# rsasaki0109/lidarslam_ros2

Hardware: AMD Instinct MI355X
Metric: scan registrations/sec (30k-pt scan vs 10-frame submap) (higher is better)
Workload: dtype f32; 1 GPU; cfg2: single NDT align(), 30000-pt VLP-32 scan (vg 0.2) vs 10-frame submap (vg 0.1), ndt_resolution 5.0, DIRECT7, max_iterations 30, transformation_epsilon 0; 1018 different scans (stream of 64); target_points=661519, voxels_valid=643, derivative_passes_last_scan=242, parallelism=1 registration stream per GPU x1, collective=none (one rank)

## Files before the change

### lidarslam_ros2_amd/csrc/ndt.hip

```cpp
#include "ndt.hpp"

#include <cmath>
#include <cstdlib>
#include <type_traits>

#include "grid_device.hpp"
#include "ndt_canon.hpp"
#include "ndt_point.hpp"
#include "sort.hpp"
#include "voxel_device.hpp"

namespace lsr {

namespace {

__host__ __device__ inline void angle_tables(const double* p, bool with_hessian, int d1_sign, float* jang, float* hang) {
  double cx, cy, cz, sx, sy, sz;
  if (fabs(p[3]) < 10e-5) { cx = 1.0; sx = 0.0; } else { cx = cos(p[3]); sx = sin(p[3]); }
  if (fabs(p[4]) < 10e-5) { cy = 1.0; sy = 0.0; } else { cy = cos(p[4]); sy = sin(p[4]); }
  if (fabs(p[5]) < 10e-5) { cz = 1.0; sz = 0.0; } else { cz = cos(p[5]); sz = sin(p[5]); }
  jang[0] = (float)(-sx * sz + cx * sy * cz); jang[1] = (float)(-sx * cz - cx * sy * sz); jang[2] = (float)(-cx * cy);
  jang[3] = (float)(cx * sz + sx * sy * cz);  jang[4] = (float)(cx * cz - sx * sy * sz);  jang[5] = (float)(-sx * cy);
  jang[6] = (float)(-sy * cz);                jang[7] = (float)(sy * sz);                 jang[8] = (float)(cy);
  jang[9] = (float)(sx * cy * cz);            jang[10] = (float)(-sx * cy * sz);          jang[11] = (float)(sx * sy);
// ... 598 lines not shown
    const long long _t3 = (long long)wall_clock64(), _c3 = (long long)clock64();         \
    unsigned long long* _r = (unsigned long long*)&g_lsr_timing[(810 + ((hess) ? 1 : 0)) * 32]; \
    atomicAdd(&_r[0], 1ull); atomicAdd(&_r[1], (unsigned long long)(_p_t1 - _p_t0)); atomicAdd(&_r[2], (unsigned long long)(_p_t2 - _p_t7)); \
    atomicAdd(&_r[3], (unsigned long long)(_t3 - _p_t2)); atomicAdd(&_r[4], (unsigned long long)(_c3 - _p_c0)); atomicAdd(&_r[5], (unsigned long long)(_t3 - _p_t0)); \
  }
#else
#define LSR_STAMP(k)
#define LSR_STAMP_T(k, t)
#define LSR_SPAN_BEGIN(seq)
#define LSR_SPAN_END(seq)
#define LSR_CTL_BEGIN(L)
#define LSR_CTL_END(col)
#define LSR_PASS_BEGIN()
#define LSR_PASS_MARK(var)
#define LSR_PASS_END(hess)
#endif

__device__ __forceinline__ int uniform_i(int v) { return __builtin_amdgcn_readfirstlane(v); }
__device__ __forceinline__ float uniform_f(float v) { return __int_as_float(__builtin_amdgcn_readfirstlane(__float_as_int(v))); }
__device__ __forceinline__ double uniform_d(double v) {
  const int lo = __builtin_amdgcn_readfirstlane(__double2loint(v)), hi = __builtin_amdgcn_readfirstlane(__double2hiint(v));
  return __hiloint2double(hi, lo);
}




__device__ __forceinline__ float dpp_quad_sum(float v) {
  v += __int_as_float(__builtin_amdgcn_update_dpp(0, __float_as_int(v), 0xB1, 0xF, 0xF, true));
  v += __int_as_float(__builtin_amdgcn_update_dpp(0, __float_as_int(v), 0x4E, 0xF, 0xF, true));
  return v;
}

template <int NOFF, int TAB, int PTS, bool KD = false>
__global__ __launch_bounds__(4 * PTS) void ndt_eval_quad_kernel(const NdtProblem P, const int seq) {
  constexpr int THREADS = 4 * PTS;
  constexpr int PITCH_PT = PTS + 8, PITCH_O = PTS + 4;
  constexpr int NT = (NOFF + 3) / 4;
  static_assert(PTS % 64 == 0, "a workgroup batch is a whole number of canonical chunks");
  if ((int)blockIdx.x >= P.nblocks) return;
  const int tid = threadIdx.x, ql = tid & 3, pq = tid >> 2;
  LSR_STAMP(0)
  LSR_STAMP_T(9, THREADS - 64)
  LSR_PASS_BEGIN()
  LSR_SPAN_BEGIN(seq)

  __shared__ float s_pt[14][PITCH_PT];
  __shared__ __attribute__((aligned(16))) float s_o[29][PITCH_O];
  __shared__ double s_bin[NDT_NBINS][32];
  __shared__ unsigned long long s_ibin[NDT_NBINS * 32];
  __shared__ double s_sum[NDT_NRED];
  __shared__ double s_lu[8][2];
  constexpr int STATE_Q = (int)(sizeof(NdtState) / 16);
  __shared__ uint4 s_state_q[STATE_Q];
  unsigned int* s_state = reinterpret_cast<unsigned int*>(s_state_q);
  extern __shared__ uint4 s_table[];

  const NdtState* __restrict__ Sin = P.st + (seq & 1);
  NdtState* __restrict__ Sout = P.st + ((seq + 1) & 1);

  const int stride = P.nblocks * PTS;
  int i = blockIdx.x * PTS + pq;
  float x = 0.f, y = 0.f, z = 0.f;
  unsigned int ang_entry = 0u, ang_entry_b = 0u;
  {
    const uint4* gq = reinterpret_cast<const uint4*>(Sin);
    const uint4 stq = (tid < STATE_Q) ? gq[tid] : make_uint4(0u, 0u, 0u, 0u);
    long long msum = 0;
    if (seq > 0 && tid < NDT_NBINS * 32) {
      const long long* b = P.bins + (size_t)((seq + 2) % NDT_NBANKS) * NDT_BANK_WORDS + tid;
      long long m[NDT_NSHARDS];
#pragma unroll
      for (int sh = 0; sh < NDT_NSHARDS; sh++) m[sh] = b[sh * (NDT_NBINS * 32)];
      msum = ((m[0] + m[1]) + (m[2] + m[3])) + ((m[4] + m[5]) + (m[6] + m[7]));
    }
    if (tid < NDT_NBINS * 32) {
      const int k = tid >> 5;
      s_bin[k][tid & 31] = canon::bin_value(msum, k);
      s_ibin[tid] = 0ull;
    }
    if (tid < STATE_Q) s_state_q[tid] = stq;
    if (i < P.n) { x = P.sx[i]; y = P.sy[i]; z = P.sz[i]; }
    if (tid < 64) ang_entry = k_angle_entries[tid];
    if (tid < 8) ang_entry_b = k_angle_entries[64 + tid];
  }
  LSR_STAMP_T(8, 0)
  LSR_STAMP_T(10, THREADS - 64)
  barrier_lds_only();
  LdsState* L = (LdsState*)s_state;
  LSR_STAMP(1)
  LSR_PASS_MARK(_p_t1)
  if (P.mailbox != nullptr && blockIdx.x == 0 && tid == 0)
    __hip_atomic_store(&P.mailbox->progress, ((unsigned long long)(unsigned int)L->token << 32) | (unsigned int)seq,
                       __ATOMIC_RELAXED, __HIP_MEMORY_SCOPE_SYSTEM);
  if (uniform_i(L->done)) {
    if (blockIdx.x == 0 && seq > 0) {
      uint4* gq = reinterpret_cast<uint4*>(Sout);
      if (tid < STATE_Q) gq[tid] = s_state_q[tid];
    }
    return;
  }
  if (TAB == NDT_TAB_LDS) {
    const int nchunks = P.lds_bytes >> 10;
    const unsigned char* img = reinterpret_cast<const unsigned char*>(P.lds_image) + (size_t)(tid & 63) * 16;
    unsigned char* dst = reinterpret_cast<unsigned char*>(s_table);
    if (tid >= 64)
      for (int c = (tid >> 6) - 1; c < nchunks; c += THREADS / 64 - 1)
        __builtin_amdgcn_global_load_lds((const __attribute__((address_space(1))) void*)(img + (size_t)c * 1024),
                                         (__attribute__((address_space(3))) void*)(dst + (size_t)c * 1024), 16, 0, 0);
  }
  if (tid < 64) {
    if (seq > 0) {
      if (tid < NDT_NRED) {
        const double b4 = s_bin[4][tid], b3 = s_bin[3][tid], b2 = s_bin[2][tid], b1 = s_bin[1][tid], b0 = s_bin[0][tid];
        double t = canon::fold(b0, b1, b2, b3, b4);
        if (s_bin[0][31] != 0.0 || s_bin[1][31] != 0.0) t = canon::poisoned();
        s_sum[tid] = t;
      }
      wave_lds_fence();
      LSR_STAMP(6)
      LSR_CTL_BEGIN(L)
      ndt_controller_wave0(L, (const LdsDouble*)s_sum);
      wave_lds_fence();
      LSR_CTL_END(0)
      LSR_STAMP(5)
      build_request_wave0(reinterpret_cast<NdtState*>(s_state), &s_lu[0][0], reinterpret_cast<float*>(&s_lu[4][0]), ang_entry, ang_entry_b);
      LSR_CTL_END(2)
      LSR_STAMP(4)
    }
    if (blockIdx.x == 0) {
      uint4* gq = reinterpret_cast<uint4*>(Sout);
      gq[tid] = s_state_q[tid];
      if (tid + 64 < STATE_Q) gq[tid + 64] = s_state_q[tid + 64];
    }
  }
  __syncthreads();
  if (uniform_i(L->done)) {
    if (P.mailbox != nullptr && blockIdx.x == 0 && tid == 0) {
      NdtMailbox* mb = P.mailbox;
#pragma unroll
      for (int k = 0; k < 16; k++) mb->final_T[k] = L->final_T[k];
      mb->converged = L->converged;
      mb->nr_iterations = L->nr_iterations;
      mb->n_evals = L->n_evals;
      mb->n_passes = L->n_passes;
      mb->trans_probability = L->trans_probability;
      mb->last_pairs = L->last_pairs;
      __threadfence_system();
      __hip_atomic_store(&mb->done, (unsigned int)L->token, __ATOMIC_RELEASE, __HIP_MEMORY_SCOPE_SYSTEM);
    }
    return;
  }
  if (blockIdx.x == 0) {
    uint4* zb = reinterpret_cast<uint4*>(P.bins + (size_t)((seq + 1) % NDT_NBANKS) * NDT_BANK_WORDS);
    for (int k = tid; k < NDT_BANK_WORDS / 2; k += THREADS) zb[k] = make_uint4(0u, 0u, 0u, 0u);
  }
  LSR_STAMP(7)
  LSR_PASS_MARK(_p_t7)

  const int form = uniform_i(L->want_hessian);
  const bool hess = form != NDT_PASS_GRAD;
  const bool fused = form == NDT_PASS_FUSED;
  const double d1d = uniform_d(L->d1);
  const float d2 = uniform_f((float)L->d2);
  float T[12];
#pragma unroll
  for (int k = 0; k < 12; k++) T[k] = uniform_f(L->T[k]);
  const float leaf = P.leaf;
  LSR_STAMP(11)

  const unsigned short* s_map = reinterpret_cast<const unsigned short*>(s_table);
  const float4* s_rec = reinterpret_cast<const float4*>(reinterpret_cast<const unsigned char*>(s_table) + P.lds_map_bytes);

  long long* const bank = P.bins + (size_t)(seq % NDT_NBANKS) * NDT_BANK_WORDS + (size_t)(blockIdx.x & (NDT_NSHARDS - 1)) * (NDT_NBINS * 32);
  const bool one_batch = (long long)blockIdx.x * PTS + stride >= (long long)P.n;
  for (int base = blockIdx.x * PTS; base < P.n; base += stride) {
    {
      const float tx = xform_ref(T[0], T[1], T[2], T[3], x, y, z);
      const float ty = xform_ref(T[4], T[5], T[6], T[7], x, y, z);
      const float tz = xform_ref(T[8], T[9], T[10], T[11], x, y, z);
      const float fx = floorf(tx / leaf), fy = floorf(ty / leaf), fz = floorf(tz / leaf);
      const bool finite_ok = (i < P.n) && (fabsf(fx) < 1.0e9f) && (fabsf(fy) < 1.0e9f) && (fabsf(fz) < 1.0e9f);
      const int ci = finite_ok ? (int)fx : INT_MIN / 2, cj = finite_ok ? (int)fy : INT_MIN / 2, ck = finite_ok ? (int)fz : INT_MIN / 2;

      bool valid[NT], score_only[NT];
      int cellv[NT];
#pragma unroll
      for (int t = 0; t < NT; t++) {
        score_only[t] = false;
        const int o = ql + 4 * t;
        int dx, dy, dz;
        Offsets<NOFF>::get(o, dx, dy, dz);
        const int a = ci + dx, b = cj + dy, c = ck + dz;
        const bool in = (o < NOFF) & (a >= P.min_b[0]) & (a <= P.max_b[0]) & (b >= P.min_b[1]) & (b <= P.max_b[1]) &
                        (c >= P.min_b[2]) & (c <= P.max_b[2]);
        valid[t] = in;
        cellv[t] = in ? ((a - P.min_b[0]) + (b - P.min_b[1]) * P.mul1 + (c - P.min_b[2]) * P.mul2) : 0;
      }
      if (KD) {
#pragma unroll
        for (int t = 0; t < NT; t++) {
          const int code = valid[t] ? P.cell_slot[cellv[t]] : -1, sl = kd_slot(code);
          const float4 cen = P.centroid[sl >= 0 ? sl : 0];
          valid[t] = (sl >= 0) & centroid_in_radius(tx, ty, tz, cen.x, cen.y, cen.z, P.radius2);
          score_only[t] = valid[t] & (code < -1);
        }
      }
      float4 r0[NT], r1[NT], r2[NT];
      if (TAB == NDT_TAB_LDS) {
        int slot[NT];
#pragma unroll
        for (int t = 0; t < NT; t++) {
          const int sl = (int)s_map[cellv[t]];
          valid[t] = valid[t] & (sl != 0xFFFF);
          slot[t] = valid[t] ? sl : 0;
        }
#pragma unroll
        for (int t = 0; t < NT; t++) {
          r0[t] = s_rec[slot[t] * 3 + 0];
          r1[t] = s_rec[slot[t] * 3 + 1];
          r2[t] = s_rec[slot[t] * 3 + 2];
        }
      } else {
        size_t ridx[NT];
#pragma unroll
        for (int t = 0; t < NT; t++) {
// ... 6 lines not shown
          }
        }
#pragma unroll
        for (int t = 0; t < NT; t++) {
          r0[t] = P.rec[ridx[t] * 4 + 0];
          r1[t] = P.rec[ridx[t] * 4 + 1];
          r2[t] = P.rec[ridx[t] * 4 + 2];
        }
      }

      if (KD) {
#pragma unroll
        for (int t = 0; t < NT; t++) {
          if (score_only[t]) {
            valid[t] = true;
            r0[t] = r1[t] = r2[t] = make_float4(0.f, 0.f, 0.f, 0.f);
          }
        }
      }
      float score = 0.f, npairs = 0.f;
      float A0 = 0.f, A1 = 0.f, A2 = 0.f;
      float E00 = 0.f, E01 = 0.f, E02 = 0.f, E11 = 0.f, E12 = 0.f, E22 = 0.f;
#pragma unroll
      for (int t = 0; t < NT; t++)
        pair_terms(valid[t], hess, tx, ty, tz, r0[t], r1[t], r2[t], d2, d1d, score, npairs, A0, A1, A2, E00, E01, E02, E11, E12, E22);
      score = dpp_quad_sum(score); npairs = dpp_quad_sum(npairs);
      A0 = dpp_quad_sum(A0); A1 = dpp_quad_sum(A1); A2 = dpp_quad_sum(A2);
      if (hess) {
        E00 = dpp_quad_sum(E00); E01 = dpp_quad_sum(E01); E02 = dpp_quad_sum(E02);
        E11 = dpp_quad_sum(E11); E12 = dpp_quad_sum(E12); E22 = dpp_quad_sum(E22);
        const float row0 = (ql == 0) ? score : (ql == 1) ? npairs : (ql == 2) ? A0 : A1;
        const float row1 = (ql == 0) ? A2 : (ql == 1) ? E00 : (ql == 2) ? E01 : E02;
        const float row2 = (ql == 0) ? E11 : (ql == 1) ? E12 : (ql == 2) ? E22 : x;
        s_pt[ql][pq] = row0;
        s_pt[4 + ql][pq] = row1;
        s_pt[8 + ql][pq] = row2;
        if (ql < 2) s_pt[12 + ql][pq] = (ql == 0) ? y : z;
      } else {
        float o[29];
        if (npairs != 0.f) {
          point_terms(false, x, y, z, score, npairs, A0, A1, A2, 0.f, 0.f, 0.f, 0.f, 0.f, 0.f, L->jang, L->hang, o);
        } else {
#pragma unroll
          for (int k = 0; k < NDT_NRED_GRAD; k++) o[k] = 0.f;
        }
        s_o[ql][pq] = (ql == 0) ? o[0] : (ql == 1) ? o[1] : (ql == 2) ? o[2] : o[3];
        s_o[4 + ql][pq] = (ql == 0) ? o[4] : (ql == 1) ? o[5] : (ql == 2) ? o[6] : o[7];
      }
      i += stride;
      x = 0.f; y = 0.f; z = 0.f;
      if (i < P.n) { x = P.sx[i]; y = P.sy[i]; z = P.sz[i]; }
    }
    LSR_STAMP(12)
    barrier_lds_only();
    if (hess) {
      if (tid < PTS) {
        const float npairs = s_pt[1][tid];
        float o[29];
        if (npairs != 0.f) {
          point_terms(true, s_pt[11][tid], s_pt[12][tid], s_pt[13][tid], s_pt[0][tid], npairs, s_pt[2][tid], s_pt[3][tid], s_pt[4][tid],
                      s_pt[5][tid], s_pt[6][tid], s_pt[7][tid], s_pt[8][tid], s_pt[9][tid], s_pt[10][tid], L->jang, L->hang, o);
        } else {
#pragma unroll
          for (int k = 0; k < 29; k++) o[k] = 0.f;
        }
#pragma unroll
        for (int k = 0; k < 29; k++) s_o[k][tid] = o[k];
      }
      LSR_STAMP(13)
      barrier_lds_only();
    }
    LSR_STAMP(14)
    if (!hess || fused) {
      constexpr int RUNS = PTS / 8;
      if (tid < NDT_NRED_GRAD * RUNS) {
        const int v = tid / RUNS, k = tid & 7;
        const double t = canon::reduce_grad(&s_o[v][8 * (tid % RUNS)]);
        bool poison;
        long long m = canon::piece(t, k < NDT_NBINS ? k : 0, &poison);
        int pz = poison ? 1 : 0;
        if (PTS == 128) { m += (long long)__shfl_xor((int)m, 8, 64); pz |= __shfl_xor(pz, 8, 64); }
        if ((tid & (RUNS - 1)) < NDT_NBINS) {
          unsigned long long* dst = one_batch ? reinterpret_cast<unsigned long long*>(bank) : s_ibin;
          if (m != 0) atomicAdd(dst + k * 32 + v, (unsigned long long)m);
          if (pz && k == 0) atomicAdd(dst + 31, 1ull);
        }
      }
    }
    if (hess) {
      constexpr int RUNS = PTS / 16;
      static_assert(NDT_NRED_GRAD * (PTS / 8) % 64 == 0 && NDT_NRED_GRAD * (PTS / 8) + (((29 - NDT_NRED_GRAD) * RUNS + 63) & ~63) <= THREADS,
                    "fused pass: the two trees sit on whole waves of their own");
      const int v0 = fused ? NDT_NRED_GRAD : 0;
      const int ht = tid - (fused ? NDT_NRED_GRAD * (PTS / 8) : 0);
      if (ht >= 0 && ht < (((29 - v0) * RUNS + 63) & ~63)) {
        const int v = v0 + ht / RUNS, sg = tid & 3;
        double t = 0.0;
        if (v < 29) t = canon::reduce_hess(&s_o[v][16 * (tid % RUNS)]);
        bool poison, poison0;
        long long m = canon::piece(t, sg + 1, &poison);
        long long m0 = canon::piece(t, 0, &poison0);
        int pz = poison0 ? 1 : 0;
        if (PTS == 128) {
          m += (long long)__shfl_xor((int)m, 4, 64); m0 += (long long)__shfl_xor((int)m0, 4, 64); pz |= __shfl_xor(pz, 4, 64);
        }
        if (v < 29 && (tid & (RUNS - 1)) < 4) {
          unsigned long long* dst = one_batch ? reinterpret_cast<unsigned long long*>(bank) : s_ibin;
          if (m != 0) atomicAdd(dst + (sg + 1) * 32 + v, (unsigned long long)m);
          if (sg == 0) {
            if (m0 != 0) atomicAdd(dst + v, (unsigned long long)m0);
            if (pz) atomicAdd(dst + 31, 1ull);
          }
        }
      }
    }
    if (!hess && base + stride < P.n) barrier_lds_only();
  }

  LSR_STAMP(2)
  LSR_PASS_MARK(_p_t2)
  if (!one_batch) {
    __syncthreads();
    if (tid < NDT_NBINS * 32) {
      const unsigned long long m = s_ibin[tid];
      if (m != 0ull) atomicAdd(reinterpret_cast<unsigned long long*>(bank + tid), m);
    }
  }
  LSR_STAMP(3)
  LSR_PASS_END(hess)
  LSR_SPAN_END(seq)
}


template <int NOFF, int TAB, int THREADS, bool BYVAL, bool SPLIT = false, bool KD = false>
__global__ __launch_bounds__(THREADS) __attribute__((amdgpu_waves_per_eu(4))) void ndt_eval_lane_kernel(const NdtProblem pv, const NdtProblem* __restrict__ probs, const int seq,
                                                                const int nb, const int tab_bytes) {
  constexpr int NWAVES = THREADS / 64;
  constexpr int PTS = SPLIT ? THREADS / 2 : THREADS;
  constexpr int NT = (NOFF + 3) / 4;
  constexpr int GROUP = 4;
  const NdtProblem& P = BYVAL ? pv : probs[blockIdx.y];
  const int tid = threadIdx.x, lane = tid & 63, wave = tid >> 6;
  if (blockIdx.x > 0 && (long long)blockIdx.x * PTS >= (long long)P.n) return;
  const int role = SPLIT ? (wave & 1) : 0;
  const int cw = SPLIT ? (wave >> 1) : wave;

  __shared__ double s_bin[NDT_NBINS][32];
  __shared__ unsigned long long s_ibin[NDT_NBINS * 32];
  __shared__ double s_sum[NDT_NRED];
  __shared__ double s_lu[8][2];
  constexpr int STATE_Q = (int)(sizeof(NdtState) / 16);
  static_assert(STATE_Q <= THREADS, "NdtState copy assumes <= THREADS uint4");
  __shared__ uint4 s_state_q[STATE_Q];
  unsigned int* s_state = reinterpret_cast<unsigned int*>(s_state_q);
  extern __shared__ uint4 s_table[];

  const NdtState* __restrict__ Sin = P.st + (seq & 1);
  NdtState* __restrict__ Sout = P.st + ((seq + 1) & 1);
// ... 63 lines not shown
      if (tid + 64 < STATE_Q) gq[tid + 64] = s_state_q[tid + 64];
    }
  }
  __syncthreads();
  if (uniform_i(L->done)) {
    if (P.mailbox != nullptr && blockIdx.x == 0 && tid == 0) {
      NdtMailbox* mb = P.mailbox;
#pragma unroll
      for (int k = 0; k < 16; k++) mb->final_T[k] = L->final_T[k];
      mb->converged = L->converged;
      mb->nr_iterations = L->nr_iterations;
      mb->n_evals = L->n_evals;
      mb->n_passes = L->n_passes;
      mb->trans_probability = L->trans_probability;
      mb->last_pairs = L->last_pairs;
      __threadfence_system();
      __hip_atomic_store(&mb->done, (unsigned int)L->token, __ATOMIC_RELEASE, __HIP_MEMORY_SCOPE_SYSTEM);
    }
    return;
  }
  if (blockIdx.x == 0) {
    uint4* zb = reinterpret_cast<uint4*>(P.bins + (size_t)((seq + 1) % NDT_NBANKS) * NDT_BANK_WORDS);
    for (int k = tid; k < NDT_BANK_WORDS / 2; k += THREADS) zb[k] = make_uint4(0u, 0u, 0u, 0u);
  }

  const int form = uniform_i(L->want_hessian);
  const bool hess = form != NDT_PASS_GRAD;
  const bool fused = form == NDT_PASS_FUSED;
  const double d1d = uniform_d(L->d1);
  const float d2 = uniform_f((float)L->d2);
  float T[12];
#pragma unroll
  for (int k = 0; k < 12; k++) T[k] = uniform_f(L->T[k]);
  const float leaf = P.leaf;
  const int mb0 = P.min_b[0], mb1 = P.min_b[1], mb2 = P.min_b[2];
  const int xb0 = P.max_b[0], xb1 = P.max_b[1], xb2 = P.max_b[2];
  const int mul1 = P.mul1, mul2 = P.mul2;
  const __attribute__((address_space(3))) unsigned short* s_map = (const __attribute__((address_space(3))) unsigned short*)s_table;
  const int map_bytes = P.lds_map_bytes;
  float* s_tile = reinterpret_cast<float*>(reinterpret_cast<unsigned char*>(s_table) + tab_bytes) + wave * canon::TILE_FLOATS;
  const GlbV4* g_rec = (const GlbV4*)P.rec;
  const GlbInt* g_cell_slot = (const GlbInt*)P.cell_slot;
  const GlbFloat* g_sx = (const GlbFloat*)P.sx;
  const GlbFloat* g_sy = (const GlbFloat*)P.sy;
  const GlbFloat* g_sz = (const GlbFloat*)P.sz;
  (void)g_rec; (void)g_cell_slot; (void)s_map; (void)map_bytes;

  for (int base = SPLIT ? blockIdx.x * PTS : blockIdx.x * PTS + cw * 64; base < n; base += stride) {
    const bool have = i < n;
    const float px = x, py = y, pz = z;
    const float tx = xform_ref(T[0], T[1], T[2], T[3], px, py, pz);
    const float ty = xform_ref(T[4], T[5], T[6], T[7], px, py, pz);
    const float tz = xform_ref(T[8], T[9], T[10], T[11], px, py, pz);
    i += stride;
    if (i < n) { x = g_sx[i]; y = g_sy[i]; z = g_sz[i]; }
    const float fx = floorf(tx / leaf), fy = floorf(ty / leaf), fz = floorf(tz / leaf);
    const bool finite_ok = have && (fabsf(fx) < 1.0e9f) && (fabsf(fy) < 1.0e9f) && (fabsf(fz) < 1.0e9f);
    const int ci = finite_ok ? (int)fx : INT_MIN / 2, cj = finite_ok ? (int)fy : INT_MIN / 2, ck = finite_ok ? (int)fz : INT_MIN / 2;
    bool inx[3], iny[3], inz[3];
#pragma unroll
    for (int d = 0; d < 3; d++) {
      inx[d] = (ci + d - 1 >= mb0) & (ci + d - 1 <= xb0);
      iny[d] = (cj + d - 1 >= mb1) & (cj + d - 1 <= xb1);
      inz[d] = (ck + d - 1 >= mb2) & (ck + d - 1 <= xb2);
    }
    const int centre = (ci - mb0) + (cj - mb1) * mul1 + (ck - mb2) * mul2;

    bool nb_ok[NOFF], nb_so[NOFF];
    int nb_rec[NOFF];
#pragma unroll
    for (int o = 0; o < NOFF; o++) {
      int dx, dy, dz;
      Offsets<NOFF>::get(o, dx, dy, dz);
      const bool in = inx[dx + 1] & iny[dy + 1] & inz[dz + 1];
      const int cell = in ? centre + dx + dy * mul1 + dz * mul2 : 0;
      nb_ok[o] = in;
      nb_so[o] = false;
      nb_rec[o] = cell;
    }
    if (KD) {
#pragma unroll
      for (int o = 0; o < NOFF; o++) {
        const int code = nb_ok[o] ? P.cell_slot[nb_rec[o]] : -1, ks = kd_slot(code);
        const float4 cen = P.centroid[ks >= 0 ? ks : 0];
        nb_ok[o] = (ks >= 0) & centroid_in_radius(tx, ty, tz, cen.x, cen.y, cen.z, P.radius2);
        nb_so[o] = nb_ok[o] & (code < -1);
      }
    }
    if (TAB == NDT_TAB_LDS) {
// ... 331 lines not shown
```

### lidarslam_ros2_amd/csrc/ndt.hpp

```cpp
#pragma once
#include "common.hpp"

namespace lsr {

enum NdtPhase : int {
  PH_INIT = 0,
  PH_MT_FIRST = 1,
  PH_MT_TRIAL = 2,
  PH_MT_HESS = 3,
  PH_DIAG = 4,
  PH_MT_LAST = 5
};

enum NdtPassForm : int {
  NDT_PASS_GRAD = 0,
  NDT_PASS_HESS = 1,
  NDT_PASS_FUSED = 2
};

constexpr int NDT_NRED = 32;
constexpr int NDT_NRED_GRAD = 8;
constexpr int NDT_LANE_THREADS = 512;
constexpr int NDT_MAX_BLOCKS = 1024;
constexpr int ndt_lane_tile_bytes(int threads) { return (threads / 64) * 16 * 68 * 4; }
// ... 32 lines not shown
  double phi_0, d_phi_0, a_l, f_l, g_l, a_u, f_u, g_u, a_t;
  int open_interval, interval_converged, step_iterations;
  int token;
  float final_T[16];
  double trans_probability;
  double last_pairs;
  int n_evals, pad1;
  int n_passes;
  int pad2[3];
};
static_assert(sizeof(NdtState) % 16 == 0 && sizeof(NdtState) <= 128 * 16, "NdtState travels as at most 128 uint4");

struct NdtMailbox {
  unsigned long long progress;
  unsigned int done;
  int converged, nr_iterations, n_evals;
  double trans_probability, last_pairs;
  float final_T[16];
  int n_passes;
};

struct NdtProblem {
  const float* sx;
  const float* sy;
  const float* sz;
  int n;
  int nblocks;
  const int* cell_slot;
  const float4* rec;
  int min_b[3];
  int max_b[3];
  int mul1, mul2;
  float leaf;
  int lds_map_bytes;
  const uint4* lds_image;
  int lds_bytes;
  long long* bins;
  NdtState* st;
  NdtMailbox* mailbox;
  const float4* centroid;
  float radius2;
};

struct NdtParamsHost {
  double resolution = 1.0, step_size = 0.1, outlier_ratio = 0.55, trans_eps = 0.1;
  int max_iterations = 35;
  int neighborhood = LSR_DIRECT7;
  int d1_sign = 1;
};

void ndt_gauss_constants(double resolution, double outlier_ratio, double* d1, double* d2);

int cloud_bbox(const DeviceCloud& cloud, float* mn, float* mx, unsigned int* n_finite, BuildScratch& sc, hipStream_t stream);
int cloud_bbox_begin(const DeviceCloud& cloud, BuildScratch& sc, hipStream_t stream);
int cloud_bbox_end(const DeviceCloud& cloud, float* mn, float* mx, unsigned int* n_finite, BuildScratch& sc, hipStream_t stream);

int ndt_build_grid(DeviceCloud& cloud, float leaf, VoxelGridDev& grid, BuildScratch& sc, hipStream_t stream);
int ndt_build_grid_end(VoxelGridDev& grid, BuildScratch& sc, hipStream_t stream);
int ndt_build_centroids(const DeviceCloud& cloud, VoxelGridDev& grid, BuildScratch& sc, hipStream_t stream);

struct NdtLaunchCfg {
  int batch = 1;
  int max_blocks = 1;
  int neighborhood = LSR_DIRECT7;
  int tab = NDT_TAB_DENSE;
  int threads = NDT_LANE_THREADS;
// ... 52 lines not shown
```

### lidarslam_ros2_amd/csrc/ndt_align.hip

```cpp
#include <algorithm>
#include <chrono>
#include <cstdlib>
#include <functional>
#include <limits>
#include <thread>

#include "api_internal.hpp"

using namespace lsr;

namespace {

int device_cus(int device) {
  static int cached[64] = {};
  if (device >= 0 && device < 64 && cached[device] > 0) return cached[device];
  int v = 0;
  if (hipDeviceGetAttribute(&v, hipDeviceAttributeMultiprocessorCount, device) != hipSuccess || v <= 0) v = 256;
  if (device >= 0 && device < 64) cached[device] = v;
  return v;
}

constexpr int NDT_LANE_SINGLE_MIN = 65536;
int ndt_resident_wgs(int device, int threads) {
  const int by_size = threads >= 1024 ? 1 : threads >= 512 ? 2 : 2048 / std::max(64, threads);
  return device_cus(device) * by_size;
}
int ndt_nblocks(size_t n, int device, int batch, int threads, int points) {
  int nb = (int)((n + points - 1) / points);
  const int share = std::max(1, ndt_resident_wgs(device, threads) / std::max(1, batch));
  nb = std::max(1, std::min(nb, std::min(share, NDT_MAX_BLOCKS)));
  return nb;
}
int cfg_wg_threads(const NdtLaunchCfg& cfg) { return cfg.quad ? 4 * cfg.threads : cfg.threads; }
int cfg_wg_points(const NdtLaunchCfg& cfg) { return (!cfg.quad && cfg.split) ? cfg.threads / 2 : cfg.threads; }

int device_lds_bytes(int device) {
  static int cached[64] = {};
  if (device >= 0 && device < 64 && cached[device] > 0) return cached[device];
  int per_block = 0, per_cu = 0;
  if (hipDeviceGetAttribute(&per_block, hipDeviceAttributeMaxSharedMemoryPerBlock, device) != hipSuccess) per_block = 0;
  if (hipDeviceGetAttribute(&per_cu, hipDeviceAttributeMaxSharedMemoryPerMultiprocessor, device) != hipSuccess) per_cu = 0;
  int v = std::max(per_block, per_cu);
  if (v <= 0) v = 64 * 1024;
  if (device >= 0 && device < 64) cached[device] = v;
  return v;
}
constexpr int NDT_QUAD_STATIC_LDS = 32 * 1024;
constexpr int NDT_LANE_STATIC_LDS = 6 * 1024;

void fill_problem(NdtProblem& P, lsr_handle h, NdtState* d_state, long long* d_bins, const NdtLaunchCfg& cfg) {
  const VoxelGridDev& g = h->target->grid;
  P.sx = h->source.x(); P.sy = h->source.y(); P.sz = h->source.z();
  P.n = (int)h->source.n;
  P.nblocks = ndt_nblocks(h->source.n, h->device, cfg.batch, cfg_wg_threads(cfg), cfg_wg_points(cfg));
  P.lds_image = g.lds_image.p;
  P.lds_map_bytes = g.lds_map_bytes;
  P.lds_bytes = g.lds_bytes;
  P.cell_slot = g.cell_slot.p;
  P.rec = g.rec.p;
  for (int k = 0; k < 3; k++) { P.min_b[k] = g.min_b[k]; P.max_b[k] = g.max_b[k]; }
  P.mul1 = g.div_b[0];
  P.mul2 = g.div_b[0] * g.div_b[1];
  P.leaf = g.leaf;
  P.st = d_state;
  P.bins = d_bins;
  P.mailbox = nullptr;
  const bool kd = h->ndt.neighborhood == LSR_KDTREE && h->target->has_centroids;
  P.centroid = kd ? g.centroid.p : nullptr;
  P.radius2 = kd ? (float)((double)(float)h->ndt.resolution * (double)(float)h->ndt.resolution) : 0.f;
}

void choose_table_mode(lsr_handle lead, lsr_handle* hs, int B, NdtLaunchCfg& cfg) {
  bool all_lds = true, all_dense = true;
  int lds_max = 0;
  for (int b = 0; b < B; b++) {
    const VoxelGridDev& g = hs[b]->target->grid;
    all_lds = all_lds && g.lds_bytes > 0;
    all_dense = all_dense && g.dense;
    lds_max = std::max(lds_max, g.lds_bytes);
  }
  const int lds_cap = device_lds_bytes(lead->device);
  const int override_mode = lead->ndt_table_mode;
  size_t n_max = 0;
  for (int b = 0; b < B; b++) n_max = std::max(n_max, hs[b]->source.n);
  const bool want_quad_single = (B == 1 && (lead->ndt_quad == 1 || (lead->ndt_quad < 0 && n_max < (size_t)NDT_LANE_SINGLE_MIN)));
  const int lane_threads = (lead->ndt_threads == 512 || lead->ndt_threads == 1024) ? lead->ndt_threads : NDT_LANE_THREADS;
  const int static_lds = want_quad_single ? NDT_QUAD_STATIC_LDS : NDT_LANE_STATIC_LDS + ndt_lane_tile_bytes(lane_threads);
  const int table_cap = std::min(want_quad_single ? NDT_LDS_TABLE_MAX_QUAD : NDT_LDS_TABLE_MAX, lds_cap - static_lds);
  const bool lds_ok = all_lds && lds_max <= table_cap;
  int tab;
  if (override_mode == NDT_TAB_COMPACT) tab = NDT_TAB_COMPACT;
  else if (override_mode == NDT_TAB_DENSE && all_dense) tab = NDT_TAB_DENSE;
  else if (override_mode == NDT_TAB_LDS && lds_ok) tab = NDT_TAB_LDS;
  else if (lds_ok) tab = NDT_TAB_LDS;
  else tab = all_dense ? NDT_TAB_DENSE : NDT_TAB_COMPACT;
  cfg.tab = tab;
// ... 525 lines not shown
```

### lidarslam_ros2_amd/csrc/ndt_canon.hpp

```cpp
#pragma once
#include <hip/hip_runtime.h>

#include "ndt.hpp"

namespace lsr {

template <int CTRL>
__device__ __forceinline__ double dpp_quad_xor(double v) {
  int lo = __double2loint(v), hi = __double2hiint(v);
  lo = __builtin_amdgcn_update_dpp(0, lo, CTRL, 0xF, 0xF, true);
  hi = __builtin_amdgcn_update_dpp(0, hi, CTRL, 0xF, 0xF, true);
  return __hiloint2double(hi, lo);
}

template <int NOFF>
struct Offsets;
template <>
struct Offsets<1> {
  static __device__ __forceinline__ void get(int o, int& dx, int& dy, int& dz) { dx = dy = dz = 0; }
};
template <>
struct Offsets<7> {
  static __device__ __forceinline__ void get(int o, int& dx, int& dy, int& dz) {
    dx = (o == 1) - (o == 2);
    dy = (o == 3) - (o == 4);
    dz = (o == 5) - (o == 6);
  }
};
template <>
struct Offsets<27> {
  static __device__ __forceinline__ void get(int o, int& dx, int& dy, int& dz) {
    dx = o / 9 - 1;
    dy = (o / 3) % 3 - 1;
    dz = o % 3 - 1;
  }
};

typedef float v4f __attribute__((ext_vector_type(4)));
typedef __attribute__((address_space(3))) const v4f LdsV4;
typedef __attribute__((address_space(1))) const v4f GlbV4;
typedef __attribute__((address_space(1))) const float GlbFloat;
typedef __attribute__((address_space(1))) const int GlbInt;

__device__ __forceinline__ void wave_lds_fence() {
  asm volatile("s_waitcnt lgkmcnt(0)" ::: "memory");
  __builtin_amdgcn_wave_barrier();
}

namespace canon {
constexpr int TILE_PITCH = 68;
constexpr int TILE_ROWS = 16;
constexpr int TILE_FLOATS = TILE_ROWS * TILE_PITCH;

__device__ __forceinline__ double quantum(const int k) { return __hiloint2double((1023 + 62 - 31 * (k + 1)) << 20, 0); }
__device__ __forceinline__ double iquantum(const int k) { return __hiloint2double((1023 - 62 + 31 * (k + 1)) << 20, 0); }

__device__ __forceinline__ int piece(const double t, const int k, bool* poison) {
  *poison = !(fabs(t) < 4611686018427387904.0);
  if (*poison) return 0;
  double r = t;
  if (k > 0) r = t - trunc(t * iquantum(k - 1)) * quantum(k - 1);
  return (int)(r * iquantum(k));
}

__device__ __forceinline__ double bin_value(const long long m, const int k) { return (double)m * quantum(k); }
__device__ __forceinline__ double fold(const double b0, const double b1, const double b2, const double b3, const double b4) {
  return (((b4 + b3) + b2) + b1) + b0;
}
__device__ __forceinline__ double poisoned() { return __longlong_as_double(0x7FF8000000000000ll); }

__device__ __forceinline__ double reduce_grad(const float* p) {
  typedef float f4 __attribute__((ext_vector_type(4)));
  const f4 a = *reinterpret_cast<const f4*>(p), b = *reinterpret_cast<const f4*>(p + 4);
  double t = (double)a.x;
  t += (double)a.y; t += (double)a.z; t += (double)a.w;
  t += (double)b.x; t += (double)b.y; t += (double)b.z; t += (double)b.w;
  t += dpp_quad_xor<0xB1>(t);
  t += dpp_quad_xor<0x4E>(t);
  t += dpp_quad_xor<0x141>(t);
  return t;
}
__device__ __forceinline__ double reduce_hess(const float* p) {
  typedef float f4 __attribute__((ext_vector_type(4)));
  const f4 a = *reinterpret_cast<const f4*>(p), b = *reinterpret_cast<const f4*>(p + 4), c = *reinterpret_cast<const f4*>(p + 8),
           d = *reinterpret_cast<const f4*>(p + 12);
  double t = (double)a.x;
  t += (double)a.y; t += (double)a.z; t += (double)a.w;
  t += (double)b.x; t += (double)b.y; t += (double)b.z; t += (double)b.w;
  t += (double)c.x; t += (double)c.y; t += (double)c.z; t += (double)c.w;
  t += (double)d.x; t += (double)d.y; t += (double)d.z; t += (double)d.w;
  t += dpp_quad_xor<0xB1>(t);
  t += dpp_quad_xor<0x4E>(t);
  return t;
}
__device__ __forceinline__ void add_piece_lds(unsigned long long* ibin, const int v, const int k, const double t) {
  bool poison;
// ... 8 lines not shown
```

### lidarslam_ros2_amd/csrc/pose_search.hip

```cpp
#include <algorithm>
#include <cmath>
#include <numeric>

#include "api_internal.hpp"
#include "ndt_canon.hpp"
#include "ndt_point.hpp"

using namespace lsr;

namespace lsr {
namespace {

template <int NOFF, int TAB>
__device__ __forceinline__ void score_point(const NdtProblem& P, const uint4* s_table, const bool have, const float px, const float py,
                                            const float pz, const float* T, const float d2, const double d1d, float& score_out,
                                            float& pairs_out) {
  constexpr int NT = (NOFF + 3) / 4;
  constexpr int GROUP = 4;
  const float tx = xform_ref(T[0], T[1], T[2], T[3], px, py, pz);
  const float ty = xform_ref(T[4], T[5], T[6], T[7], px, py, pz);
  const float tz = xform_ref(T[8], T[9], T[10], T[11], px, py, pz);
  const float leaf = P.leaf;
  const float fx = floorf(tx / leaf), fy = floorf(ty / leaf), fz = floorf(tz / leaf);
  const bool finite_ok = have && (fabsf(fx) < 1.0e9f) && (fabsf(fy) < 1.0e9f) && (fabsf(fz) < 1.0e9f);
  const int ci = finite_ok ? (int)fx : INT_MIN / 2, cj = finite_ok ? (int)fy : INT_MIN / 2, ck = finite_ok ? (int)fz : INT_MIN / 2;
  const int mb0 = P.min_b[0], mb1 = P.min_b[1], mb2 = P.min_b[2];
  const int xb0 = P.max_b[0], xb1 = P.max_b[1], xb2 = P.max_b[2];
  const int mul1 = P.mul1, mul2 = P.mul2;
  bool inx[3], iny[3], inz[3];
#pragma unroll
  for (int d = 0; d < 3; d++) {
    inx[d] = (ci + d - 1 >= mb0) & (ci + d - 1 <= xb0);
    iny[d] = (cj + d - 1 >= mb1) & (cj + d - 1 <= xb1);
    inz[d] = (ck + d - 1 >= mb2) & (ck + d - 1 <= xb2);
  }
  const int centre = (ci - mb0) + (cj - mb1) * mul1 + (ck - mb2) * mul2;
  bool nb_ok[NOFF];
  int nb_rec[NOFF];
#pragma unroll
  for (int o = 0; o < NOFF; o++) {
    int dx, dy, dz;
    Offsets<NOFF>::get(o, dx, dy, dz);
    const bool in = inx[dx + 1] & iny[dy + 1] & inz[dz + 1];
    nb_ok[o] = in;
    nb_rec[o] = in ? centre + dx + dy * mul1 + dz * mul2 : 0;
  }
  const GlbV4* g_rec = (const GlbV4*)P.rec;
  const GlbInt* g_cell_slot = (const GlbInt*)P.cell_slot;
  (void)g_rec; (void)g_cell_slot;
  if (TAB == NDT_TAB_LDS) {
    const __attribute__((address_space(3))) unsigned short* s_map = (const __attribute__((address_space(3))) unsigned short*)s_table;
    const int map_bytes = P.lds_map_bytes;
    int sl[NOFF];
#pragma unroll
    for (int o = 0; o < NOFF; o++) sl[o] = (int)s_map[nb_rec[o]];
#pragma unroll
// ... 400 lines not shown
```

### lidarslam_ros2_amd/csrc/xform_ref.hpp

```cpp
#pragma once

namespace lsr {

__device__ __forceinline__ float xform_ref(const float a, const float b, const float c, const float d, const float x, const float y,
                                           const float z) {
#pragma clang fp contract(off)
  return __fadd_rn(__fadd_rn(__fadd_rn(__fmul_rn(a, x), __fmul_rn(b, y)), __fmul_rn(c, z)), d);
}

}
```

Before: 453.6 registrations/s.

## Replace leaf division with reciprocal multiply and precompute per-thread LDS addressing

Cell indices are now computed by multiplying by a precomputed reciprocal of the leaf size. A guard falls back to exact division for the whole wave when any lane's quotient sits too close to an integer boundary, so results stay bit-identical. The eval kernel also hoists per-thread LDS and global addresses, neighbour offsets and piece quanta out of the loop, pinned in VGPRs with asm barriers. It replaces shfl_xor with DPP/ds_swizzle, uses typed address-space relaxed atomics, and reads the state T as vector loads. The aim is fewer divides, address calculations and generic-pointer atomics per pass, at the cost of more live registers and a ballot-based fallback check.

```diff
diff --git a/lidarslam_ros2_amd/csrc/ndt.hip b/lidarslam_ros2_amd/csrc/ndt.hip
--- a/lidarslam_ros2_amd/csrc/ndt.hip
+++ b/lidarslam_ros2_amd/csrc/ndt.hip
@@ -654,6 +654,18 @@
   return v;
 }
 
+typedef __attribute__((address_space(1))) unsigned long long GlbU64;
+typedef __attribute__((address_space(3))) unsigned long long LdsU64;
+typedef __attribute__((address_space(3))) float LdsF;
+typedef __attribute__((address_space(1))) unsigned char GlbByte;
+template <typename T>
+__device__ __forceinline__ void add_u64(T* p, const unsigned long long v) {
+  (void)__hip_atomic_fetch_add(p, v, __ATOMIC_RELAXED, __HIP_MEMORY_SCOPE_AGENT);
+}
+
+__device__ __forceinline__ int lane_xor8(const int v) { return __builtin_amdgcn_update_dpp(0, v, 0x128, 0xF, 0xF, true); }
+__device__ __forceinline__ int lane_xor4(const int v) { return __builtin_amdgcn_ds_swizzle(v, (4 << 10) | 0x1F); }
+
 template <int NOFF, int TAB, int PTS, bool KD = false>
 __global__ __launch_bounds__(4 * PTS) void ndt_eval_quad_kernel(const NdtProblem P, const int seq) {
   constexpr int THREADS = 4 * PTS;
@@ -685,17 +697,55 @@
   int i = blockIdx.x * PTS + pq;
   float x = 0.f, y = 0.f, z = 0.f;
   unsigned int ang_entry = 0u, ang_entry_b = 0u;
+  constexpr int RUNS_G = PTS / 8, RUNS_H = PTS / 16;
+  constexpr int FUSED_ROWS = NDT_NRED_GRAD * RUNS_G / RUNS_H - NDT_NRED_GRAD;
+  LdsF *a_so, *a_pt, *b_so;
+  const LdsF *b_pt, *g_run, *h_run;
+  LdsU64 *g_lds, *h_lds;
+  unsigned int g_off, h_off;
+  canon::PieceQ g_Q, h_Q;
+  int nb_dx[NT], nb_dy[NT], nb_dz[NT];
+  long long* bank;
   {
     const uint4* gq = reinterpret_cast<const uint4*>(Sin);
     const uint4 stq = (tid < STATE_Q) ? gq[tid] : make_uint4(0u, 0u, 0u, 0u);
-    long long msum = 0;
+    long long m[NDT_NSHARDS];
+#pragma unroll
+    for (int sh = 0; sh < NDT_NSHARDS; sh++) m[sh] = 0;
     if (seq > 0 && tid < NDT_NBINS * 32) {
       const long long* b = P.bins + (size_t)((seq + 2) % NDT_NBANKS) * NDT_BANK_WORDS + tid;
-      long long m[NDT_NSHARDS];
 #pragma unroll
       for (int sh = 0; sh < NDT_NSHARDS; sh++) m[sh] = b[sh * (NDT_NBINS * 32)];
-      msum = ((m[0] + m[1]) + (m[2] + m[3])) + ((m[4] + m[5]) + (m[6] + m[7]));
-    }
+    }
+    {
+      LdsF* const so = (LdsF*)&s_o[0][0];
+      LdsF* const pt = (LdsF*)&s_pt[0][0];
+      a_so = so + ql * PITCH_O + pq;
+      a_pt = pt + ql * PITCH_PT + pq;
+      b_pt = pt + (tid & (PTS - 1));
+      b_so = so + (tid & (PTS - 1));
+      const int gv = (tid / RUNS_G) & (NDT_NRED_GRAD - 1), gk = (tid & 7) < NDT_NBINS ? (tid & 7) : 0;
+      g_run = so + gv * PITCH_O + 8 * (tid % RUNS_G);
+      g_Q = canon::piece_q(gk);
+      g_off = (unsigned int)(gk * 32 + gv) * 8u;
+      g_lds = (LdsU64*)s_ibin + gk * 32 + gv;
+      const int hv = min(tid / RUNS_H, 28 + FUSED_ROWS), hk = (tid & 3) + 1;
+      h_run = so + hv * PITCH_O + 16 * (tid % RUNS_H);
+      h_Q = canon::piece_q(hk);
+      h_off = (unsigned int)(hk * 32 + hv) * 8u;
+      h_lds = (LdsU64*)s_ibin + hk * 32 + hv;
+#pragma unroll
+      for (int t = 0; t < NT; t++) Offsets<NOFF>::get(ql + 4 * t, nb_dx[t], nb_dy[t], nb_dz[t]);
+      bank = P.bins + (size_t)(seq % NDT_NBANKS) * NDT_BANK_WORDS + (size_t)(blockIdx.x & (NDT_NSHARDS - 1)) * (NDT_NBINS * 32);
+      asm volatile("" : "+v"(a_so), "+v"(a_pt), "+v"(b_pt), "+v"(b_so), "+v"(g_run), "+v"(h_run), "+v"(g_lds), "+v"(h_lds), "+v"(g_off), "+v"(h_off));
+      asm volatile("" : "+v"(g_Q.iq_prev), "+v"(g_Q.q_prev), "+v"(g_Q.iq), "+v"(h_Q.iq_prev), "+v"(h_Q.q_prev), "+v"(h_Q.iq));
+      if (NOFF <= 7) {
+#pragma unroll
+        for (int t = 0; t < NT; t++) asm volatile("" : "+v"(nb_dx[t]), "+v"(nb_dy[t]), "+v"(nb_dz[t]));
+      }
+      asm volatile("" : "+s"(bank));
+    }
+    const long long msum = ((m[0] + m[1]) + (m[2] + m[3])) + ((m[4] + m[5]) + (m[6] + m[7]));
     if (tid < NDT_NBINS * 32) {
       const int k = tid >> 5;
       s_bin[k][tid & 31] = canon::bin_value(msum, k);
@@ -757,7 +807,16 @@
     }
   }
   __syncthreads();
-  if (uniform_i(L->done)) {
+  const int done_w = L->done;
+  int form_w = L->want_hessian;
+  double d1_w = L->d1, d2_w = L->d2;
+  static_assert(offsetof(NdtState, T) == 0 && sizeof(NdtState) % 16 == 0, "T is read as three 16-byte vectors");
+  v4f T_q[3];
+#pragma unroll
+  for (int k = 0; k < 3; k++) T_q[k] = ((const LdsV4*)L->T)[k];
+  asm volatile("" : "+v"(form_w), "+v"(d1_w), "+v"(d2_w), "+v"(T_q[0]), "+v"(T_q[1]), "+v"(T_q[2]));
+  const float T_w[12] = {T_q[0].x, T_q[0].y, T_q[0].z, T_q[0].w, T_q[1].x, T_q[1].y, T_q[1].z, T_q[1].w, T_q[2].x, T_q[2].y, T_q[2].z, T_q[2].w};
+  if (uniform_i(done_w)) {
     if (P.mailbox != nullptr && blockIdx.x == 0 && tid == 0) {
       NdtMailbox* mb = P.mailbox;
 #pragma unroll
@@ -780,28 +839,30 @@
   LSR_STAMP(7)
   LSR_PASS_MARK(_p_t7)
 
-  const int form = uniform_i(L->want_hessian);
+  const int form = uniform_i(form_w);
   const bool hess = form != NDT_PASS_GRAD;
   const bool fused = form == NDT_PASS_FUSED;
-  const double d1d = uniform_d(L->d1);
-  const float d2 = uniform_f((float)L->d2);
+  const double d1d = uniform_d(d1_w);
+  const float d2 = uniform_f((float)d2_w);
   float T[12];
 #pragma unroll
-  for (int k = 0; k < 12; k++) T[k] = uniform_f(L->T[k]);
-  const float leaf = P.leaf;
+  for (int k = 0; k < 12; k++) T[k] = uniform_f(T_w[k]);
+  const float leaf = P.leaf, rcp_leaf = P.rcp_leaf;
   LSR_STAMP(11)
 
   const unsigned short* s_map = reinterpret_cast<const unsigned short*>(s_table);
   const float4* s_rec = reinterpret_cast<const float4*>(reinterpret_cast<const unsigned char*>(s_table) + P.lds_map_bytes);
 
-  long long* const bank = P.bins + (size_t)(seq % NDT_NBANKS) * NDT_BANK_WORDS + (size_t)(blockIdx.x & (NDT_NSHARDS - 1)) * (NDT_NBINS * 32);
   const bool one_batch = (long long)blockIdx.x * PTS + stride >= (long long)P.n;
+  GlbU64* const g_bank = (GlbU64*)bank;
+  LdsU64* const l_ibin = (LdsU64*)s_ibin;
   for (int base = blockIdx.x * PTS; base < P.n; base += stride) {
     {
       const float tx = xform_ref(T[0], T[1], T[2], T[3], x, y, z);
       const float ty = xform_ref(T[4], T[5], T[6], T[7], x, y, z);
       const float tz = xform_ref(T[8], T[9], T[10], T[11], x, y, z);
-      const float fx = floorf(tx / leaf), fy = floorf(ty / leaf), fz = floorf(tz / leaf);
+      float fx, fy, fz;
+      cell_floor3(i < P.n, tx, ty, tz, leaf, rcp_leaf, fx, fy, fz);
       const bool finite_ok = (i < P.n) && (fabsf(fx) < 1.0e9f) && (fabsf(fy) < 1.0e9f) && (fabsf(fz) < 1.0e9f);
       const int ci = finite_ok ? (int)fx : INT_MIN / 2, cj = finite_ok ? (int)fy : INT_MIN / 2, ck = finite_ok ? (int)fz : INT_MIN / 2;
 
@@ -811,9 +872,7 @@
       for (int t = 0; t < NT; t++) {
         score_only[t] = false;
         const int o = ql + 4 * t;
-        int dx, dy, dz;
-        Offsets<NOFF>::get(o, dx, dy, dz);
-        const int a = ci + dx, b = cj + dy, c = ck + dz;
+        const int a = ci + nb_dx[t], b = cj + nb_dy[t], c = ck + nb_dz[t];
         const bool in = (o < NOFF) & (a >= P.min_b[0]) & (a <= P.max_b[0]) & (b >= P.min_b[1]) & (b <= P.max_b[1]) &
                         (c >= P.min_b[2]) & (c <= P.max_b[2]);
         valid[t] = in;
@@ -886,10 +945,10 @@
         const float row0 = (ql == 0) ? score : (ql == 1) ? npairs : (ql == 2) ? A0 : A1;
         const float row1 = (ql == 0) ? A2 : (ql == 1) ? E00 : (ql == 2) ? E01 : E02;
         const float row2 = (ql == 0) ? E11 : (ql == 1) ? E12 : (ql == 2) ? E22 : x;
-        s_pt[ql][pq] = row0;
-        s_pt[4 + ql][pq] = row1;
-        s_pt[8 + ql][pq] = row2;
-        if (ql < 2) s_pt[12 + ql][pq] = (ql == 0) ? y : z;
+        a_pt[0] = row0;
+        a_pt[4 * PITCH_PT] = row1;
+        a_pt[8 * PITCH_PT] = row2;
+        if (ql < 2) a_pt[12 * PITCH_PT] = (ql == 0) ? y : z;
       } else {
         float o[29];
         if (npairs != 0.f) {
@@ -898,8 +957,8 @@
 #pragma unroll
           for (int k = 0; k < NDT_NRED_GRAD; k++) o[k] = 0.f;
         }
-        s_o[ql][pq] = (ql == 0) ? o[0] : (ql == 1) ? o[1] : (ql == 2) ? o[2] : o[3];
-        s_o[4 + ql][pq] = (ql == 0) ? o[4] : (ql == 1) ? o[5] : (ql == 2) ? o[6] : o[7];
+        a_so[0] = (ql == 0) ? o[0] : (ql == 1) ? o[1] : (ql == 2) ? o[2] : o[3];
+        a_so[4 * PITCH_O] = (ql == 0) ? o[4] : (ql == 1) ? o[5] : (ql == 2) ? o[6] : o[7];
       }
       i += stride;
       x = 0.f; y = 0.f; z = 0.f;
@@ -909,61 +968,75 @@
     barrier_lds_only();
     if (hess) {
       if (tid < PTS) {
-        const float npairs = s_pt[1][tid];
+        const float npairs = b_pt[1 * PITCH_PT];
         float o[29];
         if (npairs != 0.f) {
-          point_terms(true, s_pt[11][tid], s_pt[12][tid], s_pt[13][tid], s_pt[0][tid], npairs, s_pt[2][tid], s_pt[3][tid], s_pt[4][tid],
-                      s_pt[5][tid], s_pt[6][tid], s_pt[7][tid], s_pt[8][tid], s_pt[9][tid], s_pt[10][tid], L->jang, L->hang, o);
+          point_terms(true, b_pt[11 * PITCH_PT], b_pt[12 * PITCH_PT], b_pt[13 * PITCH_PT], b_pt[0], npairs, b_pt[2 * PITCH_PT], b_pt[3 * PITCH_PT],
+                      b_pt[4 * PITCH_PT], b_pt[5 * PITCH_PT], b_pt[6 * PITCH_PT], b_pt[7 * PITCH_PT], b_pt[8 * PITCH_PT], b_pt[9 * PITCH_PT],
+                      b_pt[10 * PITCH_PT], L->jang, L->hang, o);
         } else {
 #pragma unroll
           for (int k = 0; k < 29; k++) o[k] = 0.f;
         }
 #pragma unroll
-        for (int k = 0; k < 29; k++) s_o[k][tid] = o[k];
+        for (int k = 0; k < 29; k++) b_so[k * PITCH_O] = o[k];
       }
       LSR_STAMP(13)
       barrier_lds_only();
     }
     LSR_STAMP(14)
     if (!hess || fused) {
-      constexpr int RUNS = PTS / 8;
+      constexpr int RUNS = RUNS_G;
       if (tid < NDT_NRED_GRAD * RUNS) {
-        const int v = tid / RUNS, k = tid & 7;
-        const double t = canon::reduce_grad(&s_o[v][8 * (tid % RUNS)]);
+        const int k = tid & 7;
+        const double t = canon::reduce_grad((const float*)g_run);
         bool poison;
-        long long m = canon::piece(t, k < NDT_NBINS ? k : 0, &poison);
+        long long m = canon::piece(t, k < NDT_NBINS ? k : 0, g_Q, &poison);
         int pz = poison ? 1 : 0;
-        if (PTS == 128) { m += (long long)__shfl_xor((int)m, 8, 64); pz |= __shfl_xor(pz, 8, 64); }
+        if (PTS == 128) { m += (long long)lane_xor8((int)m); pz |= lane_xor8(pz); }
         if ((tid & (RUNS - 1)) < NDT_NBINS) {
-          unsigned long long* dst = one_batch ? reinterpret_cast<unsigned long long*>(bank) : s_ibin;
-          if (m != 0) atomicAdd(dst + k * 32 + v, (unsigned long long)m);
-          if (pz && k == 0) atomicAdd(dst + 31, 1ull);
+          if (one_batch) {
+            if (m != 0) add_u64((GlbU64*)((GlbByte*)g_bank + g_off), (unsigned long long)m);
+            if (pz && k == 0) add_u64(g_bank + 31, 1ull);
+          } else {
+            if (m != 0) add_u64(g_lds, (unsigned long long)m);
+            if (pz && k == 0) add_u64(l_ibin + 31, 1ull);
+          }
         }
       }
     }
     if (hess) {
-      constexpr int RUNS = PTS / 16;
+      constexpr int RUNS = RUNS_H;
       static_assert(NDT_NRED_GRAD * (PTS / 8) % 64 == 0 && NDT_NRED_GRAD * (PTS / 8) + (((29 - NDT_NRED_GRAD) * RUNS + 63) & ~63) <= THREADS,
                     "fused pass: the two trees sit on whole waves of their own");
       const int v0 = fused ? NDT_NRED_GRAD : 0;
       const int ht = tid - (fused ? NDT_NRED_GRAD * (PTS / 8) : 0);
       if (ht >= 0 && ht < (((29 - v0) * RUNS + 63) & ~63)) {
         const int v = v0 + ht / RUNS, sg = tid & 3;
+        const int fs = fused ? FUSED_ROWS : 0;
         double t = 0.0;
-        if (v < 29) t = canon::reduce_hess(&s_o[v][16 * (tid % RUNS)]);
+        if (v < 29) t = canon::reduce_hess((const float*)(h_run - fs * PITCH_O));
         bool poison, poison0;
-        long long m = canon::piece(t, sg + 1, &poison);
+        long long m = canon::piece(t, sg + 1, h_Q, &poison);
         long long m0 = canon::piece(t, 0, &poison0);
         int pz = poison0 ? 1 : 0;
         if (PTS == 128) {
-          m += (long long)__shfl_xor((int)m, 4, 64); m0 += (long long)__shfl_xor((int)m0, 4, 64); pz |= __shfl_xor(pz, 4, 64);
+          m += (long long)lane_xor4((int)m); m0 += (long long)lane_xor4((int)m0); pz |= lane_xor4(pz);
         }
         if (v < 29 && (tid & (RUNS - 1)) < 4) {
-          unsigned long long* dst = one_batch ? reinterpret_cast<unsigned long long*>(bank) : s_ibin;
-          if (m != 0) atomicAdd(dst + (sg + 1) * 32 + v, (unsigned long long)m);
-          if (sg == 0) {
-            if (m0 != 0) atomicAdd(dst + v, (unsigned long long)m0);
-            if (pz) atomicAdd(dst + 31, 1ull);
+          if (one_batch) {
+            GlbByte* const hb = (GlbByte*)g_bank + (h_off - 8u * (unsigned int)fs);
+            if (m != 0) add_u64((GlbU64*)hb, (unsigned long long)m);
+            if (sg == 0) {
+              if (m0 != 0) add_u64((GlbU64*)hb - 32, (unsigned long long)m0);
+              if (pz) add_u64(g_bank + 31, 1ull);
+            }
+          } else {
+            if (m != 0) add_u64(h_lds - fs, (unsigned long long)m);
+            if (sg == 0) {
+              if (m0 != 0) add_u64(h_lds - fs - 32, (unsigned long long)m0);
+              if (pz) add_u64(l_ibin + 31, 1ull);
+            }
           }
         }
       }
@@ -977,7 +1050,7 @@
     __syncthreads();
     if (tid < NDT_NBINS * 32) {
       const unsigned long long m = s_ibin[tid];
-      if (m != 0ull) atomicAdd(reinterpret_cast<unsigned long long*>(bank + tid), m);
+      if (m != 0ull) add_u64(g_bank + tid, m);
     }
   }
   LSR_STAMP(3)
@@ -1107,7 +1180,7 @@
   float T[12];
 #pragma unroll
   for (int k = 0; k < 12; k++) T[k] = uniform_f(L->T[k]);
-  const float leaf = P.leaf;
+  const float leaf = P.leaf, rcp_leaf = P.rcp_leaf;
   const int mb0 = P.min_b[0], mb1 = P.min_b[1], mb2 = P.min_b[2];
   const int xb0 = P.max_b[0], xb1 = P.max_b[1], xb2 = P.max_b[2];
   const int mul1 = P.mul1, mul2 = P.mul2;
@@ -1129,7 +1202,8 @@
     const float tz = xform_ref(T[8], T[9], T[10], T[11], px, py, pz);
     i += stride;
     if (i < n) { x = g_sx[i]; y = g_sy[i]; z = g_sz[i]; }
-    const float fx = floorf(tx / leaf), fy = floorf(ty / leaf), fz = floorf(tz / leaf);
+    float fx, fy, fz;
+    cell_floor3(have, tx, ty, tz, leaf, rcp_leaf, fx, fy, fz);
     const bool finite_ok = have && (fabsf(fx) < 1.0e9f) && (fabsf(fy) < 1.0e9f) && (fabsf(fz) < 1.0e9f);
     const int ci = finite_ok ? (int)fx : INT_MIN / 2, cj = finite_ok ? (int)fy : INT_MIN / 2, ck = finite_ok ? (int)fz : INT_MIN / 2;
     bool inx[3], iny[3], inz[3];
diff --git a/lidarslam_ros2_amd/csrc/ndt.hpp b/lidarslam_ros2_amd/csrc/ndt.hpp
--- a/lidarslam_ros2_amd/csrc/ndt.hpp
+++ b/lidarslam_ros2_amd/csrc/ndt.hpp
@@ -88,6 +88,7 @@
   int max_b[3];
   int mul1, mul2;
   float leaf;
+  float rcp_leaf;
   int lds_map_bytes;
   const uint4* lds_image;
   int lds_bytes;
diff --git a/lidarslam_ros2_amd/csrc/ndt_align.hip b/lidarslam_ros2_amd/csrc/ndt_align.hip
--- a/lidarslam_ros2_amd/csrc/ndt_align.hip
+++ b/lidarslam_ros2_amd/csrc/ndt_align.hip
@@ -6,6 +6,7 @@
 #include <thread>
 
 #include "api_internal.hpp"
+#include "xform_ref.hpp"
 
 using namespace lsr;
 
@@ -62,6 +63,7 @@
   P.mul1 = g.div_b[0];
   P.mul2 = g.div_b[0] * g.div_b[1];
   P.leaf = g.leaf;
+  P.rcp_leaf = ndt_rcp_leaf(g.leaf);
   P.st = d_state;
   P.bins = d_bins;
   P.mailbox = nullptr;
diff --git a/lidarslam_ros2_amd/csrc/ndt_canon.hpp b/lidarslam_ros2_amd/csrc/ndt_canon.hpp
--- a/lidarslam_ros2_amd/csrc/ndt_canon.hpp
+++ b/lidarslam_ros2_amd/csrc/ndt_canon.hpp
@@ -55,13 +55,18 @@
 __device__ __forceinline__ double quantum(const int k) { return __hiloint2double((1023 + 62 - 31 * (k + 1)) << 20, 0); }
 __device__ __forceinline__ double iquantum(const int k) { return __hiloint2double((1023 - 62 + 31 * (k + 1)) << 20, 0); }
 
-__device__ __forceinline__ int piece(const double t, const int k, bool* poison) {
+struct PieceQ { int iq_prev, q_prev, iq; };
+__device__ __forceinline__ PieceQ piece_q(const int k) {
+  return PieceQ{__double2hiint(iquantum(k - 1)), __double2hiint(quantum(k - 1)), __double2hiint(iquantum(k))};
+}
+__device__ __forceinline__ int piece(const double t, const int k, const PieceQ Q, bool* poison) {
   *poison = !(fabs(t) < 4611686018427387904.0);
   if (*poison) return 0;
   double r = t;
-  if (k > 0) r = t - trunc(t * iquantum(k - 1)) * quantum(k - 1);
-  return (int)(r * iquantum(k));
+  if (k > 0) r = t - trunc(t * __hiloint2double(Q.iq_prev, 0)) * __hiloint2double(Q.q_prev, 0);
+  return (int)(r * __hiloint2double(Q.iq, 0));
 }
+__device__ __forceinline__ int piece(const double t, const int k, bool* poison) { return piece(t, k, piece_q(k), poison); }
 
 __device__ __forceinline__ double bin_value(const long long m, const int k) { return (double)m * quantum(k); }
 __device__ __forceinline__ double fold(const double b0, const double b1, const double b2, const double b3, const double b4) {
diff --git a/lidarslam_ros2_amd/csrc/pose_search.hip b/lidarslam_ros2_amd/csrc/pose_search.hip
--- a/lidarslam_ros2_amd/csrc/pose_search.hip
+++ b/lidarslam_ros2_amd/csrc/pose_search.hip
@@ -20,8 +20,8 @@
   const float tx = xform_ref(T[0], T[1], T[2], T[3], px, py, pz);
   const float ty = xform_ref(T[4], T[5], T[6], T[7], px, py, pz);
   const float tz = xform_ref(T[8], T[9], T[10], T[11], px, py, pz);
-  const float leaf = P.leaf;
-  const float fx = floorf(tx / leaf), fy = floorf(ty / leaf), fz = floorf(tz / leaf);
+  float fx, fy, fz;
+  cell_floor3(have, tx, ty, tz, P.leaf, P.rcp_leaf, fx, fy, fz);
   const bool finite_ok = have && (fabsf(fx) < 1.0e9f) && (fabsf(fy) < 1.0e9f) && (fabsf(fz) < 1.0e9f);
   const int ci = finite_ok ? (int)fx : INT_MIN / 2, cj = finite_ok ? (int)fy : INT_MIN / 2, ck = finite_ok ? (int)fz : INT_MIN / 2;
   const int mb0 = P.min_b[0], mb1 = P.min_b[1], mb2 = P.min_b[2];
diff --git a/lidarslam_ros2_amd/csrc/xform_ref.hpp b/lidarslam_ros2_amd/csrc/xform_ref.hpp
--- a/lidarslam_ros2_amd/csrc/xform_ref.hpp
+++ b/lidarslam_ros2_amd/csrc/xform_ref.hpp
@@ -8,4 +8,25 @@
   return __fadd_rn(__fadd_rn(__fadd_rn(__fmul_rn(a, x), __fmul_rn(b, y)), __fmul_rn(c, z)), d);
 }
 
+inline float ndt_rcp_leaf(const float leaf) { return (leaf >= 0x1p-60f && leaf <= 0x1p60f) ? 1.0f / leaf : __builtin_nanf(""); }
+__device__ __forceinline__ bool cell_floor_fast(const float t, const float rcp_leaf, float& f) {
+#pragma clang fp contract(off)
+  const float q = __fmul_rn(t, rcp_leaf);
+  f = floorf(q);
+  return fabsf(__fadd_rn(q, -rintf(q))) > fmaxf(__fmul_rn(fabsf(q), 0x1p-21f), 0x1p-100f);
 }
+__device__ __forceinline__ float cell_floor(const float t, const float leaf, const float rcp_leaf) {
+  float f;
+  return cell_floor_fast(t, rcp_leaf, f) ? f : floorf(t / leaf);
+}
+#ifndef LSR_HOST_EMU
+__device__ __forceinline__ void cell_floor3(const bool have, const float tx, const float ty, const float tz, const float leaf,
+                                            const float rcp_leaf, float& fx, float& fy, float& fz) {
+  const bool okx = cell_floor_fast(tx, rcp_leaf, fx), oky = cell_floor_fast(ty, rcp_leaf, fy), okz = cell_floor_fast(tz, rcp_leaf, fz);
+  if (__builtin_amdgcn_ballot_w64(have && !(okx && oky && okz)) != 0ull) {
+    fx = floorf(tx / leaf); fy = floorf(ty / leaf); fz = floorf(tz / leaf);
+  }
+}
+#endif
+
+}
```

Result: faster. 470.9 registrations/s (median of 5 runs) (+3.8%).
